# gafniguy/4D-Facial-Avatars

Hardware: AMD Instinct MI355X
Metric: rays/sec at 512x512, 64 coarse + 128 fine samples (higher is better)
Workload: dtype f32

## Files before the change

4d-facial-avatars_amd/csrc/nf_mlp_bf16_dw.hip:

```cpp
#include <cstdlib>
#include <mutex>
#include <type_traits>
#include <vector>

#include "nf_mlp_bf16_common.h"
#include "nf_mlp_lcode_layout.h"
#if NFB_F16
#define NFB_DW_NAME(x) x##_f16
#else
#define NFB_DW_NAME(x) x##_bf16
#endif

struct NfbDwSeg {
    int kind;
    int sec;
    int width;
    int gs;
};
struct NfbDwTile {
    int seg, f0;
    int cs_off;
};
struct NfbDwProd {
    int na, nb, a_tile, b_tile;
// ... 154 lines not shown
}
__device__ __forceinline__ void nfb_dw_split_scaled(const float (&x)[8], float s, bf16x8& hi, bf16x8& lo) {
    unsigned hw[4], lw[4];
#pragma unroll
    for (int q = 0; q < 4; ++q) {
        unsigned h;
        float r0, r1;
        asm("v_fma_mixlo_f16 %0, %1, %2, 0 op_sel_hi:[0,0,0]" : "=v"(h) : "v"(x[2 * q]), "v"(s));
        asm("v_fma_mixhi_f16 %0, %1, %2, 0 op_sel_hi:[0,0,0]" : "+v"(h) : "v"(x[2 * q + 1]), "v"(s));
        asm("v_fma_mix_f32 %0, %1, %2, -%3 op_sel:[0,0,0] op_sel_hi:[0,0,1]" : "=v"(r0) : "v"(x[2 * q]), "v"(s), "v"(h));
        asm("v_fma_mix_f32 %0, %1, %2, -%3 op_sel:[0,0,1] op_sel_hi:[0,0,1]" : "=v"(r1) : "v"(x[2 * q + 1]), "v"(s), "v"(h));
        asm("v_cvt_pk_f16_f32 %0, %1, %2" : "=v"(lw[q]) : "v"(r0), "v"(r1));
        hw[q] = h;
    }
    typedef unsigned u32x4_t __attribute__((ext_vector_type(4)));
    hi = __builtin_bit_cast(bf16x8, (u32x4_t){hw[0], hw[1], hw[2], hw[3]});
    lo = __builtin_bit_cast(bf16x8, (u32x4_t){lw[0], lw[1], lw[2], lw[3]});
}
#endif

__device__ __forceinline__ void nfb_dw_load(__amdgpu_buffer_rsrc_t rsrc, unsigned voff, unsigned stride_b, float (&x)[8]) {
#pragma unroll
    for (int j = 0; j < 8; ++j)
        x[j] = __builtin_bit_cast(float, __builtin_amdgcn_raw_buffer_load_b32(rsrc, (int)voff, (int)(nfb_dw_point_of_slot(0, j) * stride_b), 0));
}
__device__ __forceinline__ void nfb_dw_load_tail(__amdgpu_buffer_rsrc_t rsrc, unsigned voff, unsigned stride_b, int n_ok, int h,
                                                 float (&x)[8]) {
#pragma unroll
    for (int j = 0; j < 8; ++j)
        x[j] = __builtin_bit_cast(float, __builtin_amdgcn_raw_buffer_load_b32(rsrc, (int)(nfb_dw_point_of_slot(h, j) < n_ok ? voff : 0x80000000u),
                                                                            (int)(nfb_dw_point_of_slot(0, j) * stride_b), 0));
}

template <int MODEL>
__global__ void __launch_bounds__(64 * NFB_DW_WAVES, 1)
NFB_DW_NAME(k_paper_dw_gemm)(const float* __restrict__ dz, const float* __restrict__ d_raw, const float* __restrict__ saved,
                             int64_t n_points, int64_t pts_per_slice, float* __restrict__ slabs, int slab_floats,
                             const float* __restrict__ gscale) {
    __shared__ __attribute__((aligned(16))) uint4 lds_cvt[NFB_DW_RING * NFB_DW_CVT_U4];
    const int lane = threadIdx.x & 63, wave = __builtin_amdgcn_readfirstlane(threadIdx.x >> 6);
    const int h = lane >> 5, c = lane & 31;
    const NfbDwJob& job = MODEL ? c_dwb_jobs_lcode[blockIdx.x] : c_dwb_jobs[blockIdx.x];
    const NfbDwProd pr = job.prod[wave];
    const int slice = blockIdx.y;
    const int64_t p_begin = (int64_t)slice * pts_per_slice;
    int64_t p_end = p_begin + pts_per_slice;
    if (p_end > n_points) p_end = n_points;
    const int n_stages = p_end > p_begin ? (int)((p_end - p_begin) / NFB_DW_PTS) : 0;
    const int n_tail = p_end > p_begin ? (int)(p_end - p_begin) - n_stages * NFB_DW_PTS : 0;

    const bool t_on = wave < job.ntile;
    const NfbDwTile tl = job.tile[t_on ? wave : 0];
    const NfbDwSeg tsg = job.seg[tl.seg];
    const bool t_fok = tl.f0 + c < tsg.width;
    const unsigned t_stride_b = 4u * (unsigned)tsg.width;
    const int64_t n_pad = (n_points + 31) & ~(int64_t)31;
    const bool t_stream = __builtin_amdgcn_readfirstlane((int)(t_on && tsg.kind == 3)) != 0;
    const float* t_sec = tsg.kind == 1 ? d_raw : (tsg.kind == 0 ? dz + (int64_t)tsg.sec * n_points : saved + (int64_t)tsg.sec * n_pad);
    const float* t_g = t_sec + p_begin * tsg.width;
    const __amdgpu_buffer_rsrc_t t_rsrc = t_stream
        ? __builtin_amdgcn_make_buffer_rsrc(const_cast<float*>(t_sec), (short)0, (int)((unsigned)n_pad * t_stride_b), 0x00020000)
        : __builtin_amdgcn_make_buffer_rsrc(const_cast<float*>(t_g), (short)0, (int)(n_stages * NFB_DW_PTS * t_stride_b), 0x00020000);
    const unsigned t_voff = (t_on && t_fok) ? 4u * (unsigned)(tl.f0 + c) + (unsigned)(4 * h) * t_stride_b : 0x80000000u;
    const unsigned s_blk0 = (unsigned)(p_begin >> 4) * (unsigned)(tsg.width >> 5) + (unsigned)(tl.f0 >> 5);
    const unsigned s_step = (unsigned)(tsg.width >> 5);
    const float slice_sgn = (slice & 1) ? -1.0f : 1.0f;
#if !NFB_F16
    const unsigned t_flip = (tsg.kind != 2 && (slice & 1)) ? 0x80000000u : 0u;
#endif
#if NFB_F16
    const unsigned* gbits = reinterpret_cast<const unsigned*>(gscale);
    float unused_inv;
    const float t_scale = __uint_as_float(__builtin_amdgcn_readfirstlane(
        __float_as_uint(tsg.kind == 2 ? 16.0f : slice_sgn * nfb_dw_pow2_scale(gbits[tsg.gs & 15], unused_inv))));
    const int out_gs = __builtin_amdgcn_readfirstlane(job.seg[job.tile[pr.a_tile].seg].gs & 15);
#endif
    float t_cs = 0.f;
    float xs[NFB_DW_NSET][8];
    auto load = [&](int i, float (&x)[8]) { nfb_dw_load(t_rsrc, t_voff + (unsigned)i * NFB_DW_PTS * t_stride_b, t_stride_b, x); };
    f32x16 acc[2][2];
#pragma unroll
    for (int t = 0; t < 2; ++t)
#pragma unroll
        for (int u = 0; u < 2; ++u)
#pragma unroll
            for (int r = 0; r < 16; ++r) acc[t][u][r] = 0.f;

    auto dma = [&](int i) {
        uint4* dst = lds_cvt + (i & (NFB_DW_RING - 1)) * NFB_DW_CVT_U4 + wave * 128;
        const unsigned so = (s_blk0 + (unsigned)i * s_step) * 2048u;
        __builtin_amdgcn_raw_ptr_buffer_load_lds(t_rsrc, (__attribute__((address_space(3))) void*)dst, 16, (int)(lane * 16), (int)so, 0, 0);
        __builtin_amdgcn_raw_ptr_buffer_load_lds(t_rsrc, (__attribute__((address_space(3))) void*)(dst + 64), 16, (int)(lane * 16), (int)(so + 1024u), 0, 0);
    };
    auto dma_into0 = [&](int i) {
        uint4* dst = lds_cvt + wave * 128;
        const unsigned so = (s_blk0 + (unsigned)i * s_step) * 2048u;
        __builtin_amdgcn_raw_ptr_buffer_load_lds(t_rsrc, (__attribute__((address_space(3))) void*)dst, 16, (int)(lane * 16), (int)so, 0, 0);
        __builtin_amdgcn_raw_ptr_buffer_load_lds(t_rsrc, (__attribute__((address_space(3))) void*)(dst + 64), 16, (int)(lane * 16), (int)(so + 1024u), 0, 0);
    };
    auto stage = [&](auto stream_tag, int i, const float (&xc)[8], float (&xn)[8]) {
        constexpr bool STREAM = decltype(stream_tag)::value;
        const uint4* rd = lds_cvt + ((i + NFB_DW_RING - 1) & (NFB_DW_RING - 1)) * NFB_DW_CVT_U4 + lane;
        uint4* wr = lds_cvt + (i & (NFB_DW_RING - 1)) * NFB_DW_CVT_U4 + wave * 128 + lane;
        bf16x8 ah[2], al[2], bh[2], bl[2];
#pragma unroll
        for (int t = 0; t < 2; ++t) {
            ah[t] = __builtin_bit_cast(bf16x8, rd[(pr.a_tile + t) * 128]);
            bh[t] = __builtin_bit_cast(bf16x8, rd[(pr.b_tile + t) * 128]);
        }
        __builtin_amdgcn_sched_barrier(0);
        if constexpr (!STREAM) {
            bf16x8 hi, lo;
#if NFB_F16
            t_cs += ((xc[0] + xc[1]) + (xc[2] + xc[3])) + ((xc[4] + xc[5]) + (xc[6] + xc[7]));
            nfb_dw_split_scaled(xc, t_scale, hi, lo);
#else
            t_cs += ((xc[0] + xc[1]) + (xc[2] + xc[3])) + ((xc[4] + xc[5]) + (xc[6] + xc[7]));
            float xf[8];
#pragma unroll
            for (int j = 0; j < 8; ++j) xf[j] = __uint_as_float(__float_as_uint(xc[j]) ^ t_flip);
            nfb_dw_split(xf, hi, lo);
#endif
            wr[0] = __builtin_bit_cast(uint4, hi);
            wr[64] = __builtin_bit_cast(uint4, lo);
        } else {
            dma(i + 2);
        }
        __builtin_amdgcn_sched_barrier(0);
#pragma unroll
        for (int t = 0; t < 2; ++t) bl[t] = __builtin_bit_cast(bf16x8, rd[(pr.b_tile + t) * 128 + 64]);
#pragma unroll
        for (int t = 0; t < 2; ++t)
#pragma unroll
            for (int u = 0; u < 2; ++u) acc[t][u] = NFB_MFMA(ah[t], bh[u], acc[t][u], 0, 0, 0);
        __builtin_amdgcn_sched_barrier(0);
#pragma unroll
        for (int t = 0; t < 2; ++t)
#pragma unroll
            for (int u = 0; u < 2; ++u) acc[t][u] = NFB_MFMA(ah[t], bl[u], acc[t][u], 0, 0, 0);
        __builtin_amdgcn_sched_barrier(0);
#pragma unroll
        for (int t = 0; t < 2; ++t) al[t] = __builtin_bit_cast(bf16x8, rd[(pr.a_tile + t) * 128 + 64]);
        if constexpr (!STREAM) load(i + NFB_DW_NSET - 1, xn);
        __builtin_amdgcn_sched_barrier(0);
#pragma unroll
        for (int t = 0; t < 2; ++t)
#pragma unroll
            for (int u = 0; u < 2; ++u) acc[t][u] = NFB_MFMA(al[t], bh[u], acc[t][u], 0, 0, 0);
        if constexpr (STREAM) asm volatile("s_waitcnt vmcnt(4) lgkmcnt(0)" ::: "memory");
        else asm volatile("s_waitcnt lgkmcnt(0)" ::: "memory");
        __builtin_amdgcn_s_barrier();
        asm volatile("" ::: "memory");
    };

    for (int e = threadIdx.x; e < NFB_DW_CVT_U4; e += 64 * NFB_DW_WAVES) lds_cvt[(NFB_DW_RING - 1) * NFB_DW_CVT_U4 + e] = make_uint4(0u, 0u, 0u, 0u);
    if (t_stream) {
        dma(0);
        dma(1);
        __syncthreads();
        for (int i0 = 0; i0 <= n_stages; i0 += NFB_DW_NSET) {
#pragma unroll
            for (int q = 0; q < NFB_DW_NSET; ++q) stage(std::true_type{}, i0 + q, xs[q], xs[(q + NFB_DW_NSET - 1) % NFB_DW_NSET]);
        }
    } else {
#pragma unroll
        for (int q = 0; q < NFB_DW_NSET - 1; ++q) load(q, xs[q]);
        __syncthreads();
        for (int i0 = 0; i0 <= n_stages; i0 += NFB_DW_NSET) {
#pragma unroll
            for (int q = 0; q < NFB_DW_NSET; ++q) stage(std::false_type{}, i0 + q, xs[q], xs[(q + NFB_DW_NSET - 1) % NFB_DW_NSET]);
        }
    }
    if (n_tail > 0) {
        asm volatile("s_waitcnt vmcnt(0)" ::: "memory");
        __syncthreads();
        if (t_stream) {
            dma_into0(n_stages);
        } else {
            const __amdgpu_buffer_rsrc_t rs = __builtin_amdgcn_make_buffer_rsrc(
                const_cast<float*>(t_g), (short)0, (int)((p_end - p_begin) * (int64_t)t_stride_b), 0x00020000);
            float xt[8];
            nfb_dw_load_tail(rs, t_voff + (unsigned)n_stages * NFB_DW_PTS * t_stride_b, t_stride_b, n_tail, h, xt);
            bf16x8 hi, lo;
#if NFB_F16
            t_cs += ((xt[0] + xt[1]) + (xt[2] + xt[3])) + ((xt[4] + xt[5]) + (xt[6] + xt[7]));
            nfb_dw_split_scaled(xt, t_scale, hi, lo);
#else
            t_cs += ((xt[0] + xt[1]) + (xt[2] + xt[3])) + ((xt[4] + xt[5]) + (xt[6] + xt[7]));
#pragma unroll
            for (int j = 0; j < 8; ++j) xt[j] = __uint_as_float(__float_as_uint(xt[j]) ^ t_flip);
            nfb_dw_split(xt, hi, lo);
#endif
            lds_cvt[wave * 128 + lane] = __builtin_bit_cast(uint4, hi);
            lds_cvt[wave * 128 + lane + 64] = __builtin_bit_cast(uint4, lo);
        }
        __syncthreads();
        const uint4* rd = lds_cvt + lane;
#pragma unroll
        for (int t = 0; t < 2; ++t)
#pragma unroll
            for (int u = 0; u < 2; ++u) {
                const bf16x8 ah = __builtin_bit_cast(bf16x8, rd[(pr.a_tile + t) * 128]), al = __builtin_bit_cast(bf16x8, rd[(pr.a_tile + t) * 128 + 64]);
                const bf16x8 bh = __builtin_bit_cast(bf16x8, rd[(pr.b_tile + u) * 128]), bl = __builtin_bit_cast(bf16x8, rd[(pr.b_tile + u) * 128 + 64]);
                acc[t][u] = NFB_MFMA(ah, bh, acc[t][u], 0, 0, 0);
                acc[t][u] = NFB_MFMA(ah, bl, acc[t][u], 0, 0, 0);
                acc[t][u] = NFB_MFMA(al, bh, acc[t][u], 0, 0, 0);
            }
    }

    float* slab = slabs + (int64_t)slice * slab_floats;
#if NFB_F16
    float out_scale;
    (void)nfb_dw_pow2_scale(gbits[out_gs], out_scale);
    out_scale *= slice_sgn * (1.0f / 16.0f);
#else
    const float out_scale = slice_sgn;
#endif
#pragma unroll
    for (int t = 0; t < 2; ++t) {
#pragma unroll
        for (int r = 0; r < 16; ++r) {
            const int row = 32 * t + (r & 3) + 8 * (r >> 2) + 4 * h;
            if (row >= pr.a_valid) continue;
#pragma unroll
            for (int u = 0; u < 2; ++u)
                if (32 * u + c < pr.b_valid) slab[pr.out_off + row * pr.ldo + 32 * u + c] = acc[t][u][r] * out_scale;
        }
    }
    if (t_on && tl.cs_off >= 0) {
        const float v = t_cs + __shfl_xor(t_cs, 32, 64);
        if (__lane_id() < 32 && t_fok) slab[tl.cs_off + c] = v;
    }
}

static std::mutex g_dwb_mutex;
static bool g_dwb_ready[64] = {false};

int NFB_DW_NAME(nfb_launch_dw_gemm)(int model, const float* dz, const float* d_raw, const float* saved, int64_t n_points,
                                    int64_t pts_per_slice, int n_slices, float* slabs, const float* gscale, nf_stream_t stream) {
    int dev = 0;
    hipError_t e = hipGetDevice(&dev);
    if (e != hipSuccess) return (int)e;
    if (dev < 0 || dev >= 64) return NF_EINVAL;
    {
        std::lock_guard<std::mutex> lock(g_dwb_mutex);
        if (!g_dwb_ready[dev]) {
            static NfbDwJob jobs[NFB_DW_JOBS], jobs_l[NFB_DW_JOBS_LCODE];
            nfb_build_dw_jobs(jobs);
            nfb_build_dw_jobs_lcode(jobs_l);
            e = hipMemcpyToSymbol(HIP_SYMBOL(c_dwb_jobs), jobs, sizeof(jobs));
            if (e == hipSuccess) e = hipMemcpyToSymbol(HIP_SYMBOL(c_dwb_jobs_lcode), jobs_l, sizeof(jobs_l));
            if (e != hipSuccess) return (int)e;
            g_dwb_ready[dev] = true;
        }
    }
    if (model == 0)
        hipLaunchKernelGGL((NFB_DW_NAME(k_paper_dw_gemm)<0>), dim3(NFB_DW_JOBS, (unsigned)n_slices), dim3(64 * NFB_DW_WAVES), 0, nf_s(stream),
                           dz, d_raw, saved, n_points, pts_per_slice, slabs, (int)nfl::SLAB_FLOATS, gscale);
    else
        hipLaunchKernelGGL((NFB_DW_NAME(k_paper_dw_gemm)<1>), dim3(NFB_DW_JOBS_LCODE, (unsigned)n_slices), dim3(64 * NFB_DW_WAVES), 0,
                           nf_s(stream), dz, d_raw, saved, n_points, pts_per_slice, slabs, (int)nlc::SLAB_FLOATS, gscale);
    NF_RETURN_LAUNCH();
}

#if !NFB_F16

__global__ void __launch_bounds__(256) k_unsplit_section(const unsigned short* __restrict__ stream, int64_t n_points, int width, int is_f16,
                                                         float* __restrict__ out) {
    const int64_t e = (int64_t)blockIdx.x * 256 + threadIdx.x;
    if (e >= n_points * width) return;
    const int64_t p = e / width;
    const int f = (int)(e - p * width), r = (int)(p & 15), h = (r >> 2) & 1, j = (r & 3) + 4 * (r >> 3), nt = f >> 5, c = f & 31;
    const int64_t blk = ((p >> 4) * (width >> 5) + nt) * 2;
    const int idx = (h * 32 + c) * 8 + j;
    const unsigned short bh = stream[blk * 512 + idx], bl = stream[(blk + 1) * 512 + idx];
    float v;
    if (is_f16) v = ((float)__builtin_bit_cast(_Float16, bh) + (float)__builtin_bit_cast(_Float16, bl)) * (1.0f / 16.0f);
    else v = __uint_as_float((unsigned)bh << 16) + __uint_as_float((unsigned)bl << 16);
    out[e] = v;
}

extern "C" int nf_split_saved_to_f32(int model, const float* saved_split, int64_t n_points, int is_f16, float* out, nf_stream_t stream) {
    if (!saved_split || !out || n_points <= 0 || (model != 0 && model != 1)) return NF_EINVAL;
    const int64_t n = n_points, n_pad = (n + 31) & ~(int64_t)31;
    struct Sec { int off, width, stream; };
    static const Sec paper[] = {{nfl::S_PE, 64, 0}, {nfl::S_H0, 256, 1}, {nfl::S_H1, 256, 1}, {nfl::S_H2, 256, 1}, {nfl::S_H3, 256, 1},
                                {nfl::S_H4, 256, 1}, {nfl::S_H5, 256, 1}, {nfl::S_FEAT, 256, 1}, {nfl::S_D0, 128, 1}, {nfl::S_D1, 128, 1},
                                {nfl::S_D2, 128, 1}, {nfl::S_DIRF, 16, 0}, {nfl::S_MASK, 9 * 8, 0}};
    static const Sec lcode[] = {{nlc::S_PE, 64, 0}, {nlc::S_L1, 256, 1}, {nlc::S_X0, 256, 1}, {nlc::S_X1, 256, 1}, {nlc::S_X2, 256, 1},
                                {nlc::S_FEAT, 256, 1}, {nlc::S_DIR, 128, 1}, {nlc::S_DIRF, 16, 0}, {nlc::S_MASK, 5 * 8, 0}};
    const Sec* secs = model ? lcode : paper;
    const int n_secs = model ? (int)(sizeof(lcode) / sizeof(Sec)) : (int)(sizeof(paper) / sizeof(Sec));
    for (int k = 0; k < n_secs; ++k) {
        const Sec& sc = secs[k];
        const float* src = saved_split + (int64_t)sc.off * n_pad;
        float* dst = out + (int64_t)sc.off * n;
        if (sc.stream) {
            const int64_t total = n * sc.width, grid = (total + 255) / 256;
            if (grid > 0x7fffffff) return NF_EINVAL;
            hipLaunchKernelGGL(k_unsplit_section, dim3((unsigned)grid), dim3(256), 0, nf_s(stream), reinterpret_cast<const unsigned short*>(src), n,
                               sc.width, is_f16, dst);
        } else {
            const hipError_t e = hipMemcpyAsync(dst, src, (size_t)n * sc.width * sizeof(float), hipMemcpyDeviceToDevice, nf_s(stream));
            if (e != hipSuccess) return (int)e;
        }
    }
    NF_RETURN_LAUNCH();
}

void nfb_dw_plan(int model, int64_t n_points, int64_t* pts_per_slice, int* n_slices) {
    int target = model == 0 ? 23 : 32;
    if (const char* ev = getenv("NERFACE_DW_SLICES")) { const int v = atoi(ev); if (v >= 1 && v <= 512) target = v; }
// ... 52 lines not shown
```

4d-facial-avatars_amd/csrc/nf_mlp_bf16_kernel.inc:

```
#include <type_traits>
#include "nf_mlp_bf16_machinery.inc"

__global__ void __launch_bounds__(256, 1)
NFB_KERNEL_NAME(const char* __restrict__ wstream, const float* __restrict__ cond, const float* __restrict__ ro,
                     const float* __restrict__ rd, const float* __restrict__ rd_view, const float* __restrict__ z,
                     int64_t n_points, int S, float* __restrict__ raw, float* __restrict__ saved) {
    using namespace nfl;
    constexpr bool SAVE = NFB_SAVE != 0;
    __shared__ __attribute__((aligned(16))) char lds[NFB_LDS_BYTES];
    NfbCtx cx;
    cx.lane = threadIdx.x & 63;
    cx.wave = __builtin_amdgcn_readfirstlane(threadIdx.x >> 6);
    cx.lds = lds;
    nfb_ctx_stream(cx, wstream, (unsigned)nfb::STREAM_BF16 * 2u);
    const int h = cx.lane >> 5, c = cx.lane & 31;
    const int64_t p_tile = ((int64_t)blockIdx.x * 4 + cx.wave) * 32;
    const int64_t p_raw = p_tile + c;
    const int64_t p = p_raw < n_points ? p_raw : n_points - 1;
    const float* bias = reinterpret_cast<const float*>(lds + NFB_NBUF * NFB_STAGE_BYTES);
#if NFB_F16
    const float* __restrict__ wscale = reinterpret_cast<const float*>(wstream + (size_t)nfb::STREAM_BF16 * 2);
    constexpr float ACT = (float)(1 << NFB_ACT_SHIFT);
    float wsc[2 * nfb::NL];
#pragma unroll
// ... 70 lines not shown
#pragma unroll
        for (int jj = 0; jj < 2; ++jj) {
            float sn, cs;
            nf_sincos(nf_mul(dzv, (float)(1 << (2 * h + jj))), &sn, &cs);
            x[2 * jj] = sn * ACT;
            x[2 * jj + 1] = cs * ACT;
        }
        nfb_split(x, dh, dl);
        if (SAVE && p_raw < n_points) {
            float* d = saved + (int64_t)S_DIRF * nfb_pad32(n_points) + p * 16;
            *reinterpret_cast<f32x4*>(d + 4 * (2 * h)) = (f32x4){x[0] * (1.0f / ACT), x[1] * (1.0f / ACT), 0.f, 0.f};
            *reinterpret_cast<f32x4*>(d + 4 * (2 * h + 1)) = (f32x4){x[2] * (1.0f / ACT), x[3] * (1.0f / ACT), 0.f, 0.f};
        }
    }
    nfb_wait_vm<nfb::inflight_after(-1)>();
    __builtin_amdgcn_s_barrier();
    asm volatile("" ::: "memory");
#if NFB_F16 && !NFB_EPI_OLD
    {
        float* bw = const_cast<float*>(bias);
        const int t = threadIdx.x;
#pragma unroll
        for (int l = 0; l < 7; ++l) bw[256 * l + t] *= SC(l);
        if (t < 144) bw[B_D0 + t] *= SC(7);
        if (t < 128) { bw[B_D1 + t] *= SC(8); bw[B_D2 + t] *= SC(9); }
        asm volatile("s_waitcnt lgkmcnt(0)" ::: "memory");
        __builtin_amdgcn_s_barrier();
        asm volatile("" ::: "memory");
    }
#endif

    f32x16 accA[8];
    f32x16 (&accB)[8] = accA;
#if NFB_SAVE
    bf16x8 sel[2];
    nfb_sel_operands(sel, cx.lane);
#endif
    const int64_t n_pad = nfb_pad32(n_points);
    bf16x8 th[20], tl[20];
    const bool live = p_raw < n_points;
#define NFB_FINISH(L_, acc_, NO_, RELU_, SEC_)                                                           \
    do {                                                                                                 \
         \
        if (SAVE && (RELU_) && live) nfb_save_mask<NO_>(acc_, saved + (int64_t)S_MASK * n_pad, nfb_mask_index(SEC_), n_points, p, h); \
        NFB_TO_OPERANDS(L_, acc_, NO_, RELU_);   \
    } while (0)
#if NFB_SAVE
#define NFB_RUN(L_, acc_, oh_, ol_, NOP_, prev_, PSEC_)                                                   \
    do {                                                                                                 \
        const NfbStreamTarget tg_ = nfb_stream_target(saved + (int64_t)(PSEC_) * n_pad, NOP_, p_tile, n_pad, cx.lane); \
        NFB_LAYER_STREAMING(L_, acc_, oh_, ol_, NOP_, bh, bl, sel, tg_);                                 \
    } while (0)
#else
#define NFB_RUN(L_, acc_, oh_, ol_, NOP_, prev_, PSEC_) NFB_LAYER(L_, acc_, oh_, ol_)
#endif
    nfb_init_bias<8>(accA, bias + B_L0, h, BSC(0));
    NFB_LAYER(0, accA, bh, bl);
    NFB_FINISH(0, accA, 8, true, S_H0);
#define NFB_HIDDEN_LAYER(L_, acc_, BIAS_, RELU_, SEC_, prev_, PSEC_)                 \
    do {                                                                             \
        nfb_init_bias<8>(acc_, bias + (BIAS_), h, BSC(L_));                           \
        _Pragma("unroll") for (int s = 0; s < 16; ++s) { th[s] = bh[4 + s]; tl[s] = bl[4 + s]; } \
        NFB_RUN(L_, acc_, th, tl, 8, prev_, PSEC_);                                  \
        NFB_FINISH(L_, acc_, 8, RELU_, SEC_);                                        \
    } while (0)
    NFB_HIDDEN_LAYER(1, accB, B_L1, true, S_H1, accA, S_H0);
    NFB_HIDDEN_LAYER(2, accA, B_L2, true, S_H2, accB, S_H1);
    nfb_init_bias<8>(accB, bias + B_L3, h, BSC(3));
    NFB_RUN(3, accB, bh, bl, 8, accA, S_H2);
    NFB_FINISH(3, accB, 8, true, S_H3);
    NFB_HIDDEN_LAYER(4, accA, B_L4, true, S_H4, accB, S_H3);
    NFB_HIDDEN_LAYER(5, accB, B_L5, true, S_H5, accA, S_H4);
    NFB_HIDDEN_LAYER(6, accA, B_FEAT, false, S_FEAT, accB, S_H5);
#undef NFB_HIDDEN_LAYER
    nfb_init_bias<4>(accB, bias + B_D0, h, BSC(7));
    nfb_zero(accB[4]);
    if (h == 0) accB[4][0] = bias[B_D0 + 128] * BSC(7);
#pragma unroll
    for (int s = 0; s < 16; ++s) { th[s] = bh[4 + s]; tl[s] = bl[4 + s]; }
    th[16] = dh; tl[16] = dl;
#pragma unroll
    for (int s = 17; s < nfb::KS[7]; ++s)
#pragma unroll
        for (int j = 0; j < 8; ++j) { th[s][j] = (nfb_elt)0.f; tl[s][j] = (nfb_elt)0.f; }
// ... 36 lines not shown
```

4d-facial-avatars_amd/csrc/nf_mlp_bf16_machinery.inc:

```
#ifndef NFB_KPS
#define NFB_KPS 2
#endif
#define NFB_STAGE_BYTES (NFB_KPS * 8 * 2 * 1024)
#ifndef NFB_NBUF
#define NFB_NBUF 4
#endif
#ifndef NFB_STAGGER_DIV
#define NFB_STAGGER_DIV 4
#endif
#define NFB_LA (NFB_NBUF - 1)
#define NFB_BIAS_BLOCKS 10
#define NFB_XPOSE_PITCH 144
#define NFB_XPOSE_BYTES (32 * NFB_XPOSE_PITCH)
#define NFB_XPOSE_OFF (NFB_NBUF * NFB_STAGE_BYTES + NFB_BIAS_BLOCKS * 1024)
#define NFB_LDS_BYTES (NFB_XPOSE_OFF + 4 * NFB_XPOSE_BYTES)

namespace nfb {
constexpr int stages_of(int l) { return KS[l] / NFB_KPS; }
constexpr int stage0_of(int l) { int o = 0; for (int i = 0; i < l; ++i) o += stages_of(i); return o; }
constexpr int N_STAGES = stage0_of(NL);
constexpr int layer_of_stage(int g) { int l = 0; while (l < NL && g >= stage0_of(l + 1)) ++l; return l; }
constexpr int stage_nblk(int g) { return (g < 0 || g >= N_STAGES) ? 0 : 2 * NFB_KPS * NO[layer_of_stage(g)]; }
constexpr int inflight_after(int g) { int n = 0; for (int k = 2; k <= NFB_NBUF - 1; ++k) n += stage_nblk(g + k) / 4; return n; }
constexpr int stage_blk0(int g) {
// ... 99 lines not shown
        const int k = tiles_in_stage(i);
        if (k == 0) return;
        const int region = NM / k, j = m / region;
        if (j >= k) return;
        const int r = m - j * region, d = region >= 3 ? region / 3 : 1, t = first_tile(i) + j;
        if (r == 0) {
            __builtin_amdgcn_sched_barrier(0);
            nfb_tile_to_slab(slab, sv[t], lane);
            __builtin_amdgcn_sched_barrier(0);
        } else if (r == d) {
            __builtin_amdgcn_sched_barrier(0);
            nfb_slab_to_transit(slab, tr, lane);
            __builtin_amdgcn_sched_barrier(0);
        } else if (r == 2 * d) {
            __builtin_amdgcn_sched_barrier(0);
            nfb_transit_to_global<32 * NOP>(tr, tg, t);
            __builtin_amdgcn_sched_barrier(0);
        }
    }
};
template <int NOP>
__device__ __forceinline__ void nfb_save_now(const f32x16 (&sv)[8], const NfbSaveTarget& tg, char* slab, int lane) {
#pragma unroll
    for (int t = 0; t < NOP; ++t) {
        f32x4 tr[4];
        nfb_tile_to_slab(slab, sv[t], lane);
        __builtin_amdgcn_wave_barrier();
        nfb_slab_to_transit(slab, tr, lane);
        nfb_transit_to_global<32 * NOP>(tr, tg, t);
        __builtin_amdgcn_wave_barrier();
    }
}

__device__ __forceinline__ void nfb_sel_operands(bf16x8 (&sel)[2], int lane) {
    const int h = lane >> 5, c = lane & 31;
#pragma unroll
    for (int u = 0; u < 2; ++u)
#pragma unroll
        for (int j = 0; j < 8; ++j) sel[u][j] = (nfb_elt)((c == 16 * u + 4 * h + (j & 3) + 8 * (j >> 2)) ? 1.0f : 0.0f);
}
struct NfbStreamTarget {
    __amdgpu_buffer_rsrc_t rsrc;
    unsigned voff;
};
__device__ __forceinline__ NfbStreamTarget nfb_stream_target(float* sec, int n_tiles, int64_t p_tile, int64_t n_pad, int lane) {
    NfbStreamTarget t;
    t.rsrc = __builtin_amdgcn_make_buffer_rsrc(sec, (short)0, (int)((unsigned)n_pad * (unsigned)(128 * n_tiles)), 0x00020000);
    t.voff = (unsigned)(p_tile >> 4) * (unsigned)(2048 * n_tiles) + (unsigned)lane * 16u;
    return t;
}
template <int NOP, int NST, int OFF>
struct NfbStreamSide {
    const bf16x8 (&oh)[20];
    const bf16x8 (&ol)[20];
    const bf16x8 (&sel)[2];
    NfbStreamTarget tg;
    f32x16 dh;
    static constexpr int TPS = (NOP + NST - 1) / NST;
    static constexpr int first_tile(int i) { return i * TPS < NOP ? i * TPS : NOP; }
    static constexpr int tiles_in_stage(int i) { return (i < 0 || i >= NST) ? 0 : first_tile(i + 1) - first_tile(i); }
    static constexpr int stores_in_stage(int i) { return 4 * tiles_in_stage(i); }
    __device__ __forceinline__ NfbStreamSide(const bf16x8 (&oh_)[20], const bf16x8 (&ol_)[20], const bf16x8 (&sel_)[2], const NfbStreamTarget& tg_)
        : oh(oh_), ol(ol_), sel(sel_), tg(tg_) {}
    __device__ __forceinline__ void xpose(const bf16x8 (&o)[20], int t, int part) {
        __builtin_amdgcn_sched_barrier(0);
        if (part == 0) {
            f32x16 z;
#pragma unroll
            for (int q = 0; q < 16; ++q) z[q] = 0.0f;
            dh = NFB_MFMA(o[OFF + 2 * t], sel[0], z, 0, 0, 0);
        } else {
            dh = NFB_MFMA(o[OFF + 2 * t + 1], sel[1], dh, 0, 0, 0);
        }
        __builtin_amdgcn_sched_barrier(0);
    }
    __device__ __forceinline__ void flush(int t, int hl) {
        __builtin_amdgcn_sched_barrier(0);
#pragma unroll
        for (int u = 0; u < 2; ++u) {
            bf16x8 f;
#pragma unroll
            for (int q = 0; q < 8; ++q) f[q] = (nfb_elt)dh[8 * u + q];
            __builtin_amdgcn_raw_buffer_store_b128(__builtin_bit_cast(nfb_u32x4, f), tg.rsrc, (int)tg.voff, ((u * NOP + t) * 2 + hl) * 1024, NFB_SAVE_AUX);
        }
        __builtin_amdgcn_sched_barrier(0);
    }
    __device__ __forceinline__ void at(int i, int m, int NM) {
        const int k = tiles_in_stage(i);
        if (k == 0) return;
        const int region = NM / k, j = m / region;
        if (j >= k) return;
        const int r = m - j * region, d = region >= 6 ? region / 3 : 2, t = first_tile(i) + j;
        if (r == 0) xpose(oh, t, 0);
        else if (r == 1) xpose(oh, t, 1);
        else if (r == d) { flush(t, 0); xpose(ol, t, 0); }
        else if (r == d + 1) xpose(ol, t, 1);
        else if (r == 2 * d) flush(t, 1);
    }
};
#define NFB_LAYER_STREAMING(L_, acc_, bh_, bl_, NOP_, oh_, ol_, sel_, tg_)                                              \
    do {                                                                                                                \
        typedef NfbStreamSide<NOP_, nfb::stages_of(L_), 4> side_t_;                                                     \
        side_t_ side_(oh_, ol_, sel_, tg_);                                                                             \
        nfb_layer<nfb::stage0_of(L_), nfb::stages_of(L_), nfb::NO[L_], 0, side_t_>(cx, acc_, bh_, bl_, side_);         \
    } while (0)

template <int G, int NO, int I = 0, class SIDE = NfbNoSide, int PM = 7>
__device__ __forceinline__ void nfb_stage(const NfbCtx& cx, f32x16 (&acc)[8], const bf16x8 (&bh)[20], const bf16x8 (&bl)[20], int s0, SIDE& side) {
    constexpr int nb2 = nfb::stage_nblk(G + NFB_LA);
    constexpr int blk2 = nfb::stage_blk0(G + NFB_LA);
    constexpr int off2 = ((G + NFB_LA) % NFB_NBUF) * NFB_STAGE_BYTES;
    constexpr int NM = NFB_KPS * ((PM & 1) + ((PM >> 1) & 1) + ((PM >> 2) & 1)) * NO;
    const char* base = cx.lds + (G % NFB_NBUF) * NFB_STAGE_BYTES + cx.lane * 16;
    int m = 0;
#ifndef NFB_TILE_GROUP
#define NFB_TILE_GROUP 8
#endif
    constexpr int TG = NO < NFB_TILE_GROUP ? NO : NFB_TILE_GROUP;
#pragma unroll
    for (int u = 0; u < NFB_KPS; ++u) {
#pragma unroll
        for (int n0 = 0; n0 < NO; n0 += TG) {
            bf16x8 ah[TG], al[TG];
#pragma unroll
            for (int nt = 0; nt < TG; ++nt) {
                ah[nt] = *reinterpret_cast<const bf16x8*>(base + ((u * NO + n0 + nt) * 2 + 0) * 1024);
                al[nt] = *reinterpret_cast<const bf16x8*>(base + ((u * NO + n0 + nt) * 2 + 1) * 1024);
            }
#pragma unroll
            for (int t = 0; t < 3; ++t)
#pragma unroll
                for (int nt = 0; nt < TG; ++nt) {
                    if (!((PM >> t) & 1)) continue;
#ifndef NFB_NO_DMA
#define NFB_NO_DMA 0
#endif
// ... 169 lines not shown
```

4d-facial-avatars_amd/csrc/nf_mlp_lcode_bf16_kernel.inc:

```
#include <type_traits>
#include "nf_mlp_bf16_machinery.inc"

__global__ void __launch_bounds__(256, 1)
NFB_KERNEL_NAME(const char* __restrict__ wstream, const float* __restrict__ cond, const float* __restrict__ ro,
                const float* __restrict__ rd, const float* __restrict__ rd_view, const float* __restrict__ z, int64_t n_points, int S,
                float* __restrict__ raw, float* __restrict__ saved) {
    using namespace nlc;
    constexpr bool SAVE = NFB_SAVE != 0;
    __shared__ __attribute__((aligned(16))) char lds[NFB_LDS_BYTES];
    NfbCtx cx;
    cx.lane = threadIdx.x & 63;
    cx.wave = __builtin_amdgcn_readfirstlane(threadIdx.x >> 6);
    cx.lds = lds;
    nfb_ctx_stream(cx, wstream, (unsigned)nfb::STREAM_BF16 * 2u);
    const int h = cx.lane >> 5, c = cx.lane & 31;
    const int64_t p_tile = ((int64_t)blockIdx.x * 4 + cx.wave) * 32;
    const int64_t p_raw = p_tile + c;
    const int64_t p = p_raw < n_points ? p_raw : n_points - 1;
    const float* bias = reinterpret_cast<const float*>(lds + NFB_NBUF * NFB_STAGE_BYTES);
#if NFB_F16
    const float* __restrict__ wscale = reinterpret_cast<const float*>(wstream + (size_t)nfb::STREAM_BF16 * 2);
    constexpr float ACT = (float)(1 << NFB_ACT_SHIFT);
    float wsc[2 * nfb::NL];
#pragma unroll
// ... 73 lines not shown
            nf_sincos(nf_mul(dzv, (float)(1 << (2 * h + jj))), &sn, &cs);
            x[2 * jj] = sn * ACT;
            x[2 * jj + 1] = cs * ACT;
        }
        nfb_split(x, dh, dl);
        if (SAVE && p_raw < n_points) {
            float* d = saved + (int64_t)S_DIRF * nfb_pad32(n_points) + p * 16;
            *reinterpret_cast<f32x4*>(d + 4 * (2 * h)) = (f32x4){x[0] * (1.0f / ACT), x[1] * (1.0f / ACT), 0.f, 0.f};
            *reinterpret_cast<f32x4*>(d + 4 * (2 * h + 1)) = (f32x4){x[2] * (1.0f / ACT), x[3] * (1.0f / ACT), 0.f, 0.f};
        }
    }
    nfb_wait_vm<nfb::inflight_after(-1)>();
    __builtin_amdgcn_s_barrier();
    asm volatile("" ::: "memory");
#if NFB_F16 && !NFB_EPI_OLD
    {
        float* bw = const_cast<float*>(bias);
        const int t = threadIdx.x;
        bw[B_L1 + t] *= SC(0);
        bw[B_X0 + t] *= SC(1);
        bw[B_X1 + t] *= SC(2);
        bw[B_X2 + t] *= SC(3);
        bw[B_FEAT + t] *= SC(5);
        if (t < 16) bw[B_ALPHA + t] *= SC(4);
        if (t < 128) bw[B_DIR + t] *= SC(6);
        asm volatile("s_waitcnt lgkmcnt(0)" ::: "memory");
        __builtin_amdgcn_s_barrier();
        asm volatile("" ::: "memory");
    }
#endif

    f32x16 accA[8];
    f32x16 (&accB)[8] = accA;
#if NFB_SAVE
    bf16x8 sel[2];
    nfb_sel_operands(sel, cx.lane);
#endif
    const int64_t n_pad = nfb_pad32(n_points);
    bf16x8 th[20], tl[20];
    const bool live = p_raw < n_points;
#define NFB_LC_FINISH(L_, acc_, NO_, RELU_, MASK_)                                                       \
    do {                                                                                                 \
         \
        if (SAVE && (RELU_) && live) nfb_save_mask<NO_>(acc_, saved + (int64_t)S_MASK * n_pad, MASK_, n_points, p, h); \
        NFB_TO_OPERANDS(L_, acc_, NO_, RELU_);                                                           \
    } while (0)
#if NFB_SAVE
#define NFB_LC_RUN(L_, acc_, oh_, ol_, NOP_, prev_, PSEC_)                                               \
    do {                                                                                                 \
        const NfbStreamTarget tg_ = nfb_stream_target(saved + (int64_t)(PSEC_) * n_pad, NOP_, p_tile, n_pad, cx.lane); \
        NFB_LAYER_STREAMING(L_, acc_, oh_, ol_, NOP_, bh, bl, sel, tg_);                                 \
    } while (0)
#else
#define NFB_LC_RUN(L_, acc_, oh_, ol_, NOP_, prev_, PSEC_) NFB_LAYER(L_, acc_, oh_, ol_)
#endif
    nfb_init_bias<8>(accA, bias + B_L1, h, BSC(0));
    NFB_LAYER(0, accA, bh, bl);
    NFB_LC_FINISH(0, accA, 8, false, 0);
#define NFB_LC_HIDDEN(L_, acc_, BIAS_, MASK_, prev_, PSEC_)                          \
    do {                                                                             \
        nfb_init_bias<8>(acc_, bias + (BIAS_), h, BSC(L_));                           \
        _Pragma("unroll") for (int s = 0; s < 16; ++s) { th[s] = bh[4 + s]; tl[s] = bl[4 + s]; } \
        NFB_LC_RUN(L_, acc_, th, tl, 8, prev_, PSEC_);                               \
        NFB_LC_FINISH(L_, acc_, 8, true, MASK_);                                     \
    } while (0)
    NFB_LC_HIDDEN(1, accB, B_X0, 0, accA, S_L1);
    NFB_LC_HIDDEN(2, accA, B_X1, 1, accB, S_X0);
    NFB_LC_HIDDEN(3, accB, B_X2, 2, accA, S_X1);
#pragma unroll
    for (int s = 0; s < 16; ++s) { th[s] = bh[4 + s]; tl[s] = bl[4 + s]; }
    nfb_zero(accA[0]);
    if (h == 0) accA[0][0] = bias[B_ALPHA] * BSC(4);
    NFB_LAYER(4, accA, th, tl);
    const float sigma_raw = accA[0][0] * OUT_INV(4);
    nfb_init_bias<8>(accA, bias + B_FEAT, h, BSC(5));
    NFB_LC_RUN(5, accA, th, tl, 8, accB, S_X2);
    NFB_LC_FINISH(5, accA, 8, true, 3);
#undef NFB_LC_HIDDEN
    nfb_init_bias<4>(accB, bias + B_DIR, h, BSC(6));
#pragma unroll
    for (int s = 0; s < 16; ++s) { th[s] = bh[4 + s]; tl[s] = bl[4 + s]; }
    th[16] = dh; tl[16] = dl;
#pragma unroll
    for (int s = 17; s < nfb::KS[6]; ++s)
// ... 27 lines not shown
```

Baseline: 572,200.

## Store saved activations untransposed and read them with LDS transpose loads

The forward kernel previously transposed saved activation tiles with selector MFMAs before streaming them to memory. It now stores the operand fragments directly in a new layout. The weight-gradient kernel compensates by reading those streamed B tiles through ds_read_b64_tr_b16 transpose loads, and the split-to-f32 decoder is updated to the new layout. This removes MFMA and conversion work from the forward save path, at the cost of a second templated path in the dw kernel and more inline asm with a manual lgkmcnt wait.

```diff
diff --git a/4d-facial-avatars_amd/csrc/nf_mlp_bf16_dw.hip b/4d-facial-avatars_amd/csrc/nf_mlp_bf16_dw.hip
--- a/4d-facial-avatars_amd/csrc/nf_mlp_bf16_dw.hip
+++ b/4d-facial-avatars_amd/csrc/nf_mlp_bf16_dw.hip
@@ -210,6 +210,20 @@
                                                                             (int)(nfb_dw_point_of_slot(0, j) * stride_b), 0));
 }
 
+__device__ __forceinline__ unsigned nfb_dw_tr_lane_off(int lane) {
+    const unsigned h = (unsigned)lane >> 5, c = (unsigned)lane & 31u;
+    return 256u * h + 128u * (c >> 4) + 32u * ((c >> 2) & 3u) + 16u * (c & 1u) + 8u * ((c >> 1) & 1u);
+}
+typedef short nfb_s16x4 __attribute__((ext_vector_type(4)));
+template <int OFF>
+__device__ __forceinline__ bf16x8 nfb_dw_read_tr(unsigned addr) {
+    nfb_s16x4 r0, r1;
+    asm volatile("ds_read_b64_tr_b16 %0, %2 offset:%3\n\tds_read_b64_tr_b16 %1, %2 offset:%4" : "=v"(r0), "=v"(r1) : "v"(addr), "n"(OFF), "n"(OFF + 512)
+                 : "memory");
+    return __builtin_bit_cast(bf16x8, __builtin_shufflevector(r0, r1, 0, 1, 2, 3, 4, 5, 6, 7));
+}
+__device__ __forceinline__ void nfb_dw_wait_tr(bf16x8 (&f)[2]) { asm volatile("s_waitcnt lgkmcnt(0)" : "+v"(f[0]), "+v"(f[1]) :: "memory"); }
+
 template <int MODEL>
 __global__ void __launch_bounds__(64 * NFB_DW_WAVES, 1)
 NFB_DW_NAME(k_paper_dw_gemm)(const float* __restrict__ dz, const float* __restrict__ d_raw, const float* __restrict__ saved,
@@ -242,6 +256,8 @@
     const unsigned t_voff = (t_on && t_fok) ? 4u * (unsigned)(tl.f0 + c) + (unsigned)(4 * h) * t_stride_b : 0x80000000u;
     const unsigned s_blk0 = (unsigned)(p_begin >> 4) * (unsigned)(tsg.width >> 5) + (unsigned)(tl.f0 >> 5);
     const unsigned s_step = (unsigned)(tsg.width >> 5);
+    const bool b_tr = __builtin_amdgcn_readfirstlane((int)(job.seg[job.tile[pr.b_tile].seg].kind == 3)) != 0;
+    const unsigned b_tr_off = (unsigned)pr.b_tile * 2048u + nfb_dw_tr_lane_off(lane);
     const float slice_sgn = (slice & 1) ? -1.0f : 1.0f;
 #if !NFB_F16
     const unsigned t_flip = (tsg.kind != 2 && (slice & 1)) ? 0x80000000u : 0u;
@@ -276,15 +292,26 @@
         __builtin_amdgcn_raw_ptr_buffer_load_lds(t_rsrc, (__attribute__((address_space(3))) void*)dst, 16, (int)(lane * 16), (int)so, 0, 0);
         __builtin_amdgcn_raw_ptr_buffer_load_lds(t_rsrc, (__attribute__((address_space(3))) void*)(dst + 64), 16, (int)(lane * 16), (int)(so + 1024u), 0, 0);
     };
-    auto stage = [&](auto stream_tag, int i, const float (&xc)[8], float (&xn)[8]) {
-        constexpr bool STREAM = decltype(stream_tag)::value;
-        const uint4* rd = lds_cvt + ((i + NFB_DW_RING - 1) & (NFB_DW_RING - 1)) * NFB_DW_CVT_U4 + lane;
+    auto read_b_tr = [&](auto hl_tag, const uint4* buf, bf16x8 (&b)[2]) {
+        constexpr int HL = decltype(hl_tag)::value;
+        const unsigned a = (unsigned)(size_t)(__attribute__((address_space(3))) const char*)buf + b_tr_off;
+        b[0] = nfb_dw_read_tr<HL * 1024>(a);
+        b[1] = nfb_dw_read_tr<2048 + HL * 1024>(a);
+        __builtin_amdgcn_sched_barrier(0);
+    };
+    using hi_t = std::integral_constant<int, 0>;
+    using lo_t = std::integral_constant<int, 1>;
+    auto stage = [&](auto stream_tag, auto btr_tag, int i, const float (&xc)[8], float (&xn)[8]) {
+        constexpr bool STREAM = decltype(stream_tag)::value, BTR = decltype(btr_tag)::value;
+        const uint4* rb = lds_cvt + ((i + NFB_DW_RING - 1) & (NFB_DW_RING - 1)) * NFB_DW_CVT_U4;
+        const uint4* rd = rb + lane;
         uint4* wr = lds_cvt + (i & (NFB_DW_RING - 1)) * NFB_DW_CVT_U4 + wave * 128 + lane;
         bf16x8 ah[2], al[2], bh[2], bl[2];
+        if constexpr (BTR) read_b_tr(hi_t{}, rb, bh);
 #pragma unroll
         for (int t = 0; t < 2; ++t) {
             ah[t] = __builtin_bit_cast(bf16x8, rd[(pr.a_tile + t) * 128]);
-            bh[t] = __builtin_bit_cast(bf16x8, rd[(pr.b_tile + t) * 128]);
+            if constexpr (!BTR) bh[t] = __builtin_bit_cast(bf16x8, rd[(pr.b_tile + t) * 128]);
         }
         __builtin_amdgcn_sched_barrier(0);
         if constexpr (!STREAM) {
@@ -306,12 +333,15 @@
         }
         __builtin_amdgcn_sched_barrier(0);
 #pragma unroll
-        for (int t = 0; t < 2; ++t) bl[t] = __builtin_bit_cast(bf16x8, rd[(pr.b_tile + t) * 128 + 64]);
+        for (int t = 0; t < 2; ++t)
+            if constexpr (!BTR) bl[t] = __builtin_bit_cast(bf16x8, rd[(pr.b_tile + t) * 128 + 64]);
+        if constexpr (BTR) read_b_tr(lo_t{}, rb, bl);
 #pragma unroll
         for (int t = 0; t < 2; ++t)
 #pragma unroll
             for (int u = 0; u < 2; ++u) acc[t][u] = NFB_MFMA(ah[t], bh[u], acc[t][u], 0, 0, 0);
         __builtin_amdgcn_sched_barrier(0);
+        if constexpr (BTR) nfb_dw_wait_tr(bl);
 #pragma unroll
         for (int t = 0; t < 2; ++t)
 #pragma unroll
@@ -332,59 +362,74 @@
     };
 
     for (int e = threadIdx.x; e < NFB_DW_CVT_U4; e += 64 * NFB_DW_WAVES) lds_cvt[(NFB_DW_RING - 1) * NFB_DW_CVT_U4 + e] = make_uint4(0u, 0u, 0u, 0u);
-    if (t_stream) {
-        dma(0);
-        dma(1);
-        __syncthreads();
-        for (int i0 = 0; i0 <= n_stages; i0 += NFB_DW_NSET) {
-#pragma unroll
-            for (int q = 0; q < NFB_DW_NSET; ++q) stage(std::true_type{}, i0 + q, xs[q], xs[(q + NFB_DW_NSET - 1) % NFB_DW_NSET]);
-        }
-    } else {
-#pragma unroll
-        for (int q = 0; q < NFB_DW_NSET - 1; ++q) load(q, xs[q]);
-        __syncthreads();
-        for (int i0 = 0; i0 <= n_stages; i0 += NFB_DW_NSET) {
-#pragma unroll
-            for (int q = 0; q < NFB_DW_NSET; ++q) stage(std::false_type{}, i0 + q, xs[q], xs[(q + NFB_DW_NSET - 1) % NFB_DW_NSET]);
-        }
-    }
-    if (n_tail > 0) {
-        asm volatile("s_waitcnt vmcnt(0)" ::: "memory");
-        __syncthreads();
+    auto run = [&](auto btr_tag) {
         if (t_stream) {
-            dma_into0(n_stages);
+            dma(0);
+            dma(1);
+            __syncthreads();
+            for (int i0 = 0; i0 <= n_stages; i0 += NFB_DW_NSET) {
+#pragma unroll
+                for (int q = 0; q < NFB_DW_NSET; ++q) stage(std::true_type{}, btr_tag, i0 + q, xs[q], xs[(q + NFB_DW_NSET - 1) % NFB_DW_NSET]);
+            }
         } else {
-            const __amdgpu_buffer_rsrc_t rs = __builtin_amdgcn_make_buffer_rsrc(
-                const_cast<float*>(t_g), (short)0, (int)((p_end - p_begin) * (int64_t)t_stride_b), 0x00020000);
-            float xt[8];
-            nfb_dw_load_tail(rs, t_voff + (unsigned)n_stages * NFB_DW_PTS * t_stride_b, t_stride_b, n_tail, h, xt);
-            bf16x8 hi, lo;
+#pragma unroll
+            for (int q = 0; q < NFB_DW_NSET - 1; ++q) load(q, xs[q]);
+            __syncthreads();
+            for (int i0 = 0; i0 <= n_stages; i0 += NFB_DW_NSET) {
+#pragma unroll
+                for (int q = 0; q < NFB_DW_NSET; ++q) stage(std::false_type{}, btr_tag, i0 + q, xs[q], xs[(q + NFB_DW_NSET - 1) % NFB_DW_NSET]);
+            }
+        }
+        if (n_tail > 0) {
+            asm volatile("s_waitcnt vmcnt(0)" ::: "memory");
+            __syncthreads();
+            if (t_stream) {
+                dma_into0(n_stages);
+            } else {
+                const __amdgpu_buffer_rsrc_t rs = __builtin_amdgcn_make_buffer_rsrc(
+                    const_cast<float*>(t_g), (short)0, (int)((p_end - p_begin) * (int64_t)t_stride_b), 0x00020000);
+                float xt[8];
+                nfb_dw_load_tail(rs, t_voff + (unsigned)n_stages * NFB_DW_PTS * t_stride_b, t_stride_b, n_tail, h, xt);
+                bf16x8 hi, lo;
 #if NFB_F16
-            t_cs += ((xt[0] + xt[1]) + (xt[2] + xt[3])) + ((xt[4] + xt[5]) + (xt[6] + xt[7]));
-            nfb_dw_split_scaled(xt, t_scale, hi, lo);
+                t_cs += ((xt[0] + xt[1]) + (xt[2] + xt[3])) + ((xt[4] + xt[5]) + (xt[6] + xt[7]));
+                nfb_dw_split_scaled(xt, t_scale, hi, lo);
 #else
-            t_cs += ((xt[0] + xt[1]) + (xt[2] + xt[3])) + ((xt[4] + xt[5]) + (xt[6] + xt[7]));
-#pragma unroll
-            for (int j = 0; j < 8; ++j) xt[j] = __uint_as_float(__float_as_uint(xt[j]) ^ t_flip);
-            nfb_dw_split(xt, hi, lo);
-#endif
-            lds_cvt[wave * 128 + lane] = __builtin_bit_cast(uint4, hi);
-            lds_cvt[wave * 128 + lane + 64] = __builtin_bit_cast(uint4, lo);
-        }
-        __syncthreads();
-        const uint4* rd = lds_cvt + lane;
-#pragma unroll
-        for (int t = 0; t < 2; ++t)
-#pragma unroll
-            for (int u = 0; u < 2; ++u) {
-                const bf16x8 ah = __builtin_bit_cast(bf16x8, rd[(pr.a_tile + t) * 128]), al = __builtin_bit_cast(bf16x8, rd[(pr.a_tile + t) * 128 + 64]);
-                const bf16x8 bh = __builtin_bit_cast(bf16x8, rd[(pr.b_tile + u) * 128]), bl = __builtin_bit_cast(bf16x8, rd[(pr.b_tile + u) * 128 + 64]);
-                acc[t][u] = NFB_MFMA(ah, bh, acc[t][u], 0, 0, 0);
-                acc[t][u] = NFB_MFMA(ah, bl, acc[t][u], 0, 0, 0);
-                acc[t][u] = NFB_MFMA(al, bh, acc[t][u], 0, 0, 0);
+                t_cs += ((xt[0] + xt[1]) + (xt[2] + xt[3])) + ((xt[4] + xt[5]) + (xt[6] + xt[7]));
+#pragma unroll
+                for (int j = 0; j < 8; ++j) xt[j] = __uint_as_float(__float_as_uint(xt[j]) ^ t_flip);
+                nfb_dw_split(xt, hi, lo);
+#endif
+                lds_cvt[wave * 128 + lane] = __builtin_bit_cast(uint4, hi);
+                lds_cvt[wave * 128 + lane + 64] = __builtin_bit_cast(uint4, lo);
             }
-    }
+            __syncthreads();
+            const uint4* rd = lds_cvt + lane;
+            bf16x8 bh[2], bl[2];
+            if constexpr (decltype(btr_tag)::value) {
+                read_b_tr(hi_t{}, lds_cvt, bh);
+                read_b_tr(lo_t{}, lds_cvt, bl);
+                nfb_dw_wait_tr(bl);
+            }
+#pragma unroll
+            for (int u = 0; u < 2; ++u)
+                if constexpr (!decltype(btr_tag)::value) {
+                    bh[u] = __builtin_bit_cast(bf16x8, rd[(pr.b_tile + u) * 128]);
+                    bl[u] = __builtin_bit_cast(bf16x8, rd[(pr.b_tile + u) * 128 + 64]);
+                }
+#pragma unroll
+            for (int t = 0; t < 2; ++t)
+#pragma unroll
+                for (int u = 0; u < 2; ++u) {
+                    const bf16x8 ah = __builtin_bit_cast(bf16x8, rd[(pr.a_tile + t) * 128]), al = __builtin_bit_cast(bf16x8, rd[(pr.a_tile + t) * 128 + 64]);
+                    acc[t][u] = NFB_MFMA(ah, bh[u], acc[t][u], 0, 0, 0);
+                    acc[t][u] = NFB_MFMA(ah, bl[u], acc[t][u], 0, 0, 0);
+                    acc[t][u] = NFB_MFMA(al, bh[u], acc[t][u], 0, 0, 0);
+                }
+        }
+    };
+    if (b_tr) run(std::true_type{});
+    else run(std::false_type{});
 
     float* slab = slabs + (int64_t)slice * slab_floats;
 #if NFB_F16
@@ -448,14 +493,15 @@
     const int64_t e = (int64_t)blockIdx.x * 256 + threadIdx.x;
     if (e >= n_points * width) return;
     const int64_t p = e / width;
-    const int f = (int)(e - p * width), r = (int)(p & 15), h = (r >> 2) & 1, j = (r & 3) + 4 * (r >> 3), nt = f >> 5, c = f & 31;
+    const int f = (int)(e - p * width), P = (int)(p & 15), nt = f >> 5, c = f & 31;
     const int64_t blk = ((p >> 4) * (width >> 5) + nt) * 2;
-    const int idx = (h * 32 + c) * 8 + j;
+    const int chunk = 16 * (P >> 2) + 8 * (c >> 4) + 2 * (P & 3) + ((c >> 2) & 1);
+    const int idx = chunk * 8 + 4 * ((c >> 3) & 1) + (c & 3);
     const unsigned short bh = stream[blk * 512 + idx], bl = stream[(blk + 1) * 512 + idx];
     float v;
     if (is_f16) v = ((float)__builtin_bit_cast(_Float16, bh) + (float)__builtin_bit_cast(_Float16, bl)) * (1.0f / 16.0f);
     else v = __uint_as_float((unsigned)bh << 16) + __uint_as_float((unsigned)bl << 16);
-    out[e] = v;
+    out[e] = v + 0.0f;
 }
 
 extern "C" int nf_split_saved_to_f32(int model, const float* saved_split, int64_t n_points, int is_f16, float* out, nf_stream_t stream) {
diff --git a/4d-facial-avatars_amd/csrc/nf_mlp_bf16_kernel.inc b/4d-facial-avatars_amd/csrc/nf_mlp_bf16_kernel.inc
--- a/4d-facial-avatars_amd/csrc/nf_mlp_bf16_kernel.inc
+++ b/4d-facial-avatars_amd/csrc/nf_mlp_bf16_kernel.inc
@@ -126,10 +126,6 @@
 
     f32x16 accA[8];
     f32x16 (&accB)[8] = accA;
-#if NFB_SAVE
-    bf16x8 sel[2];
-    nfb_sel_operands(sel, cx.lane);
-#endif
     const int64_t n_pad = nfb_pad32(n_points);
     bf16x8 th[20], tl[20];
     const bool live = p_raw < n_points;
@@ -143,7 +139,7 @@
 #define NFB_RUN(L_, acc_, oh_, ol_, NOP_, prev_, PSEC_)                                                   \
     do {                                                                                                 \
         const NfbStreamTarget tg_ = nfb_stream_target(saved + (int64_t)(PSEC_) * n_pad, NOP_, p_tile, n_pad, cx.lane); \
-        NFB_LAYER_STREAMING(L_, acc_, oh_, ol_, NOP_, bh, bl, sel, tg_);                                 \
+        NFB_LAYER_STREAMING(L_, acc_, oh_, ol_, NOP_, bh, bl, tg_);                                      \
     } while (0)
 #else
 #define NFB_RUN(L_, acc_, oh_, ol_, NOP_, prev_, PSEC_) NFB_LAYER(L_, acc_, oh_, ol_)
diff --git a/4d-facial-avatars_amd/csrc/nf_mlp_bf16_machinery.inc b/4d-facial-avatars_amd/csrc/nf_mlp_bf16_machinery.inc
--- a/4d-facial-avatars_amd/csrc/nf_mlp_bf16_machinery.inc
+++ b/4d-facial-avatars_amd/csrc/nf_mlp_bf16_machinery.inc
@@ -155,57 +155,33 @@
     }
 }
 
-__device__ __forceinline__ void nfb_sel_operands(bf16x8 (&sel)[2], int lane) {
-    const int h = lane >> 5, c = lane & 31;
-#pragma unroll
-    for (int u = 0; u < 2; ++u)
-#pragma unroll
-        for (int j = 0; j < 8; ++j) sel[u][j] = (nfb_elt)((c == 16 * u + 4 * h + (j & 3) + 8 * (j >> 2)) ? 1.0f : 0.0f);
-}
 struct NfbStreamTarget {
     __amdgpu_buffer_rsrc_t rsrc;
     unsigned voff;
 };
 __device__ __forceinline__ NfbStreamTarget nfb_stream_target(float* sec, int n_tiles, int64_t p_tile, int64_t n_pad, int lane) {
     NfbStreamTarget t;
+    const unsigned h = (unsigned)lane >> 5, c = (unsigned)lane & 31u;
     t.rsrc = __builtin_amdgcn_make_buffer_rsrc(sec, (short)0, (int)((unsigned)n_pad * (unsigned)(128 * n_tiles)), 0x00020000);
-    t.voff = (unsigned)(p_tile >> 4) * (unsigned)(2048 * n_tiles) + (unsigned)lane * 16u;
+    t.voff = ((unsigned)(p_tile >> 4) + (c >> 4)) * (unsigned)(2048 * n_tiles) + 16u * (16u * ((c >> 2) & 3u) + 2u * (c & 3u) + h);
     return t;
 }
 template <int NOP, int NST, int OFF>
 struct NfbStreamSide {
     const bf16x8 (&oh)[20];
     const bf16x8 (&ol)[20];
-    const bf16x8 (&sel)[2];
     NfbStreamTarget tg;
-    f32x16 dh;
     static constexpr int TPS = (NOP + NST - 1) / NST;
     static constexpr int first_tile(int i) { return i * TPS < NOP ? i * TPS : NOP; }
     static constexpr int tiles_in_stage(int i) { return (i < 0 || i >= NST) ? 0 : first_tile(i + 1) - first_tile(i); }
     static constexpr int stores_in_stage(int i) { return 4 * tiles_in_stage(i); }
-    __device__ __forceinline__ NfbStreamSide(const bf16x8 (&oh_)[20], const bf16x8 (&ol_)[20], const bf16x8 (&sel_)[2], const NfbStreamTarget& tg_)
-        : oh(oh_), ol(ol_), sel(sel_), tg(tg_) {}
-    __device__ __forceinline__ void xpose(const bf16x8 (&o)[20], int t, int part) {
+    __device__ __forceinline__ NfbStreamSide(const bf16x8 (&oh_)[20], const bf16x8 (&ol_)[20], const NfbStreamTarget& tg_)
+        : oh(oh_), ol(ol_), tg(tg_) {}
+    __device__ __forceinline__ void store(int t, int q) {
+        const int u = q & 1, hl = q >> 1;
+        const bf16x8& f = hl ? ol[OFF + 2 * t + u] : oh[OFF + 2 * t + u];
         __builtin_amdgcn_sched_barrier(0);
-        if (part == 0) {
-            f32x16 z;
-#pragma unroll
-            for (int q = 0; q < 16; ++q) z[q] = 0.0f;
-            dh = NFB_MFMA(o[OFF + 2 * t], sel[0], z, 0, 0, 0);
-        } else {
-            dh = NFB_MFMA(o[OFF + 2 * t + 1], sel[1], dh, 0, 0, 0);
-        }
-        __builtin_amdgcn_sched_barrier(0);
-    }
-    __device__ __forceinline__ void flush(int t, int hl) {
-        __builtin_amdgcn_sched_barrier(0);
-#pragma unroll
-        for (int u = 0; u < 2; ++u) {
-            bf16x8 f;
-#pragma unroll
-            for (int q = 0; q < 8; ++q) f[q] = (nfb_elt)dh[8 * u + q];
-            __builtin_amdgcn_raw_buffer_store_b128(__builtin_bit_cast(nfb_u32x4, f), tg.rsrc, (int)tg.voff, ((u * NOP + t) * 2 + hl) * 1024, NFB_SAVE_AUX);
-        }
+        __builtin_amdgcn_raw_buffer_store_b128(__builtin_bit_cast(nfb_u32x4, f), tg.rsrc, (int)tg.voff, (2 * t + hl) * 1024 + 128 * u, NFB_SAVE_AUX);
         __builtin_amdgcn_sched_barrier(0);
     }
     __device__ __forceinline__ void at(int i, int m, int NM) {
@@ -213,18 +189,19 @@
         if (k == 0) return;
         const int region = NM / k, j = m / region;
         if (j >= k) return;
-        const int r = m - j * region, d = region >= 6 ? region / 3 : 2, t = first_tile(i) + j;
-        if (r == 0) xpose(oh, t, 0);
-        else if (r == 1) xpose(oh, t, 1);
-        else if (r == d) { flush(t, 0); xpose(ol, t, 0); }
-        else if (r == d + 1) xpose(ol, t, 1);
-        else if (r == 2 * d) flush(t, 1);
-    }
-};
-#define NFB_LAYER_STREAMING(L_, acc_, bh_, bl_, NOP_, oh_, ol_, sel_, tg_)                                              \
+        const int r = m - j * region, t = first_tile(i) + j;
+        if (region < 4) {
+            if (r == 0)
+                for (int q = 0; q < 4; ++q) store(t, q);
+        } else if (r % (region / 4) == 0 && r / (region / 4) < 4) {
+            store(t, r / (region / 4));
+        }
+    }
+};
+#define NFB_LAYER_STREAMING(L_, acc_, bh_, bl_, NOP_, oh_, ol_, tg_)                                                    \
     do {                                                                                                                \
         typedef NfbStreamSide<NOP_, nfb::stages_of(L_), 4> side_t_;                                                     \
-        side_t_ side_(oh_, ol_, sel_, tg_);                                                                             \
+        side_t_ side_(oh_, ol_, tg_);                                                                                   \
         nfb_layer<nfb::stage0_of(L_), nfb::stages_of(L_), nfb::NO[L_], 0, side_t_>(cx, acc_, bh_, bl_, side_);         \
     } while (0)
 
diff --git a/4d-facial-avatars_amd/csrc/nf_mlp_lcode_bf16_kernel.inc b/4d-facial-avatars_amd/csrc/nf_mlp_lcode_bf16_kernel.inc
--- a/4d-facial-avatars_amd/csrc/nf_mlp_lcode_bf16_kernel.inc
+++ b/4d-facial-avatars_amd/csrc/nf_mlp_lcode_bf16_kernel.inc
@@ -129,10 +129,6 @@
 
     f32x16 accA[8];
     f32x16 (&accB)[8] = accA;
-#if NFB_SAVE
-    bf16x8 sel[2];
-    nfb_sel_operands(sel, cx.lane);
-#endif
     const int64_t n_pad = nfb_pad32(n_points);
     bf16x8 th[20], tl[20];
     const bool live = p_raw < n_points;
@@ -146,7 +142,7 @@
 #define NFB_LC_RUN(L_, acc_, oh_, ol_, NOP_, prev_, PSEC_)                                               \
     do {                                                                                                 \
         const NfbStreamTarget tg_ = nfb_stream_target(saved + (int64_t)(PSEC_) * n_pad, NOP_, p_tile, n_pad, cx.lane); \
-        NFB_LAYER_STREAMING(L_, acc_, oh_, ol_, NOP_, bh, bl, sel, tg_);                                 \
+        NFB_LAYER_STREAMING(L_, acc_, oh_, ol_, NOP_, bh, bl, tg_);                                      \
     } while (0)
 #else
 #define NFB_LC_RUN(L_, acc_, oh_, ol_, NOP_, prev_, PSEC_) NFB_LAYER(L_, acc_, oh_, ol_)
```

Result: no change. 572,400, median of 6 (+0.0%).
